# PythonOptimizers/pysparse

Measured on AMD Instinct MI355X. Metric: CSR SpMV GB/s (7-pt Poisson, % of 8 TB/s HBM peak) + PCG iters/s, higher is better.
Workload: dtype f64

## Files before the change

### pysparse_amd/csrc/psp_csr_kernels.h

```cpp

constexpr int kBlock = 256;


__global__ void build_chunk_table(int nrows, const int *__restrict__ ind, int target, int nchunks,
                                  int2 *__restrict__ tab) {
  int c = blockIdx.x * blockDim.x + threadIdx.x;
  if (c > nchunks) return;
  int r;
  if (c == nchunks) {
    r = nrows;
  } else {
    long want = (long)c * target;
    int lo = 0, hi = nrows;
    while (lo < hi) {
      int mid = lo + ((hi - lo) >> 1);
      if ((long)ind[mid] >= want)
        hi = mid;
      else
        lo = mid + 1;
    }
    r = lo;
  }
  tab[c] = make_int2(r, ind[r]);
}
// ... 1526 lines not shown
  const int blk = blk0 + vb * 4 + wid;
  const long r = (long)blk * kDiaRows + 2 * lane;
  double dsum = 0.0;
  if (blk < blk1 && r < nrows) {
    const uint2 mm = *reinterpret_cast<const uint2 *>(mask + r);
    const unsigned m0 = mm.x, m1 = mm.y;
    const double *vp = valT + (size_t)blk * NO * kDiaRows + 2 * lane;
    const long cmax = (long)ncols - 2;
    double a0 = 0.0, a1 = 0.0;
#pragma unroll
    for (int g = 0; g < NO; g += 8) {
      constexpr int G = 8;
      d2v v[G], xv[G];
      bool edge = false;
#pragma unroll
      for (int u = 0; u < G; ++u) {
        if (g + u < NO) {
          v[u] = ldg<true>(reinterpret_cast<const d2v *>(vp + (g + u) * kDiaRows));
          const long c = r + offs.o[g + u];
          const long cc = c < 0 ? 0 : (c > cmax ? cmax : c);
          const d2u t = *reinterpret_cast<const d2u *>(x + cc);
          xv[u].x = t.x;
          xv[u].y = t.y;
          edge |= cc != c;
        }
      }
      if (edge) {
#pragma unroll
        for (int u = 0; u < G; ++u) {
          if (g + u < NO) {
            const long c = r + offs.o[g + u];
            if (c < 0 || c > cmax) {
              xv[u].x = (c >= 0 && c < ncols) ? x[c] : 0.0;
              xv[u].y = (c + 1 >= 0 && c + 1 < ncols) ? x[c + 1] : 0.0;
            }
          }
        }
      }
#pragma unroll
      for (int u = 0; u < G; ++u) {
        if (g + u < NO) {
          const double t0 = a0 + v[u].x * xv[u].x;
          const double t1 = a1 + v[u].y * xv[u].y;
          a0 = ((m0 >> (g + u)) & 1u) ? t0 : a0;
          a1 = ((m1 >> (g + u)) & 1u) ? t1 : a1;
        }
      }
    }
    if (r + 1 < nrows) {
      d2u outu;
      outu.x = a0;
      outu.y = a1;
      __builtin_nontemporal_store(outu, reinterpret_cast<d2u *>(y + r));
      if (dotv) {
        const d2u u = *reinterpret_cast<const d2u *>(dotv + r);
        dsum += u.x * a0;
        dsum += u.y * a1;
      }
    } else {
      y[r] = a0;
      if (dotv) dsum += dotv[r] * a0;
    }
  }
  if (partials) {
    dsum = wave_sum(dsum);
    if (lane == 0) red[wid] = dsum;
    __syncthreads();
    if (threadIdx.x == 0) partials[blockIdx.x] = red[0] + red[1] + red[2] + red[3];
  }
}

__global__ __launch_bounds__(256) void csr_spmv_w4y(
    int blk0, int blk1, int nrows, int ncols, int stripe, int no, const int *__restrict__ offs,
    const double *__restrict__ valT, const unsigned long long *__restrict__ mask, const double *__restrict__ x,
    double *__restrict__ y, const double *__restrict__ dotv, double *__restrict__ partials,
    const int *__restrict__ skip) {
  if (skip && *skip) return;
  __shared__ double red[4];
  const int lane = threadIdx.x & 63;
  const int wid = __builtin_amdgcn_readfirstlane(threadIdx.x >> 6);
  int vb = (int)blockIdx.x;
  if (stripe > 0) {
    const int k = vb >> 3;
    vb = ((k / stripe) * 8 + (vb & 7)) * stripe + k % stripe;
  }
  const int blk = blk0 + vb * 4 + wid;
  const long r = (long)blk * kDiaRows + 2 * lane;
  double dsum = 0.0;
  if (blk < blk1 && r < nrows) {
    const ulonglong2 mm = *reinterpret_cast<const ulonglong2 *>(mask + r);
    const unsigned long long m0 = mm.x, m1 = mm.y;
    const double *vp = valT + (size_t)blk * no * kDiaRows + 2 * lane;
    const long cmax = (long)ncols - 2;
    double a0 = 0.0, a1 = 0.0;
    for (int g = 0; g < no; g += 8) {
      constexpr int G = 8;
      d2v v[G], xv[G];
      int og[G];
      bool edge = false;
#pragma unroll
      for (int u = 0; u < G; ++u) {
        const int gu = g + u < no ? g + u : no - 1;
        og[u] = offs[gu];
        v[u] = ldg<true>(reinterpret_cast<const d2v *>(vp + (size_t)gu * kDiaRows));
        const long c = r + og[u];
        const long cc = c < 0 ? 0 : (c > cmax ? cmax : c);
        const d2u t = *reinterpret_cast<const d2u *>(x + cc);
        xv[u].x = t.x;
        xv[u].y = t.y;
        edge |= cc != c;
      }
      if (edge) {
#pragma unroll
        for (int u = 0; u < G; ++u) {
          const long c = r + og[u];
          if (c < 0 || c > cmax) {
            xv[u].x = (c >= 0 && c < ncols) ? x[c] : 0.0;
            xv[u].y = (c + 1 >= 0 && c + 1 < ncols) ? x[c + 1] : 0.0;
          }
        }
      }
#pragma unroll
      for (int u = 0; u < G; ++u) {
        const double t0 = a0 + v[u].x * xv[u].x;
        const double t1 = a1 + v[u].y * xv[u].y;
        const bool live = g + u < no;
        a0 = (live && ((m0 >> (g + u)) & 1ull)) ? t0 : a0;
        a1 = (live && ((m1 >> (g + u)) & 1ull)) ? t1 : a1;
      }
    }
    if (r + 1 < nrows) {
      d2u outu;
      outu.x = a0;
      outu.y = a1;
      __builtin_nontemporal_store(outu, reinterpret_cast<d2u *>(y + r));
      if (dotv) {
        const d2u u = *reinterpret_cast<const d2u *>(dotv + r);
        dsum += u.x * a0;
        dsum += u.y * a1;
      }
    } else {
      y[r] = a0;
      if (dotv) dsum += dotv[r] * a0;
    }
  }
  if (partials) {
    dsum = wave_sum(dsum);
    if (lane == 0) red[wid] = dsum;
    __syncthreads();
    if (threadIdx.x == 0) partials[blockIdx.x] = red[0] + red[1] + red[2] + red[3];
  }
}

template <int NO, int PRE, bool XU = false>
__global__ __launch_bounds__(256) void csr_spmv_w4_pf(
    int nrows, int stripe, DiaOffs offs, const double *__restrict__ valT,
    const unsigned short *__restrict__ mask, const double *__restrict__ r, const double *__restrict__ dinv,
    double dc, const double *__restrict__ p_old, double *__restrict__ p_new, double *__restrict__ q,
    double beta, int first, double *__restrict__ partials, const psp::PcgDev *__restrict__ dstate,
    double *__restrict__ x = nullptr, double *__restrict__ scan_partials = nullptr) {
  double alpha_x = 0.0;
  bool xp = false;
  if (dstate) {
    if (dstate->status) return;
    beta = dstate->beta;
    first = dstate->it == 1;
    if constexpr (XU) {
      alpha_x = dstate->alpha_x;
      xp = dstate->xpend != 0;
    }
  }
  __shared__ double red[4];
  __shared__ double red2[4];
  double dmax = 0.0;
  const int lane = threadIdx.x & 63;
  const int wid = __builtin_amdgcn_readfirstlane(threadIdx.x >> 6);
  int vb = (int)blockIdx.x;
  if (stripe > 0) {
    const int k = vb >> 3;
    vb = ((k / stripe) * 8 + (vb & 7)) * stripe + k % stripe;
  }
  const int blk = vb * 4 + wid;
  const long row = (long)blk * kDiaRows + 2 * lane;
  double dsum = 0.0;
  if (row < nrows) {
    const unsigned mm = *reinterpret_cast<const unsigned *>(mask + row);
    const unsigned m0 = mm & 0xffffu, m1 = mm >> 16;
    const double *vp = valT + (size_t)blk * NO * kDiaRows + 2 * lane;
    d2v v[NO];
#pragma unroll
    for (int o = 0; o < NO; ++o) v[o] = ldg<true>(reinterpret_cast<const d2v *>(vp + o * kDiaRows));
    const long cmax = (long)nrows - 2;
    const long rc = row > cmax ? cmax : row;
    d2u rr[NO + 1], pp[NO + 1], dd[NO + 1];
    bool edge = rc != row;
#pragma unroll
    for (int o = 0; o <= NO; ++o) {
      const long c = o < NO ? row + offs.o[o] : row;
      const long cc = c < 0 ? 0 : (c > cmax ? cmax : c);
      rr[o] = *reinterpret_cast<const d2u *>(r + cc);
      if (!first) pp[o] = *reinterpret_cast<const d2u *>(p_old + cc);
      if constexpr (PRE == 1) dd[o] = *reinterpret_cast<const d2u *>(dinv + cc);
      edge |= cc != c;
    }
    if (edge) {
#pragma unroll
      for (int o = 0; o <= NO; ++o) {
        const long c = o < NO ? row + offs.o[o] : row;
        if (c < 0 || c > cmax) {
          const bool i0 = c >= 0 && c < nrows, i1 = c + 1 >= 0 && c + 1 < nrows;
          rr[o].x = i0 ? r[c] : 0.0;
          rr[o].y = i1 ? r[c + 1] : 0.0;
          if (!first) {
            pp[o].x = i0 ? p_old[c] : 0.0;
            pp[o].y = i1 ? p_old[c + 1] : 0.0;
          }
          if constexpr (PRE == 1) {
            dd[o].x = i0 ? dinv[c] : 0.0;
            dd[o].y = i1 ? dinv[c + 1] : 0.0;
          }
        }
      }
    }
    d2v pn[NO + 1];
#pragma unroll
    for (int o = 0; o <= NO; ++o) {
      double z0 = rr[o].x, z1 = rr[o].y;
      if constexpr (PRE == 1) {
        z0 = z0 * dd[o].x;
        z1 = z1 * dd[o].y;
      }
      if constexpr (PRE == 2) {
        z0 = z0 * dc;
        z1 = z1 * dc;
      }
      if (!first) {
        z0 = z0 + beta * pp[o].x;
        z1 = z1 + beta * pp[o].y;
      }
      pn[o].x = z0;
      pn[o].y = z1;
    }
    double a0 = 0.0, a1 = 0.0;
#pragma unroll
    for (int o = 0; o < NO; ++o) {
      const double t0 = a0 + v[o].x * pn[o].x;
      const double t1 = a1 + v[o].y * pn[o].y;
      a0 = ((m0 >> o) & 1u) ? t0 : a0;
      a1 = ((m1 >> o) & 1u) ? t1 : a1;
    }
    if (row + 1 < nrows) {
      d2u outq, outp;
      outq.x = a0;
      outq.y = a1;
      outp.x = pn[NO].x;
      outp.y = pn[NO].y;
      __builtin_nontemporal_store(outq, reinterpret_cast<d2u *>(q + row));
      *reinterpret_cast<d2u *>(p_new + row) = outp;
      dsum += pn[NO].x * a0;
      dsum += pn[NO].y * a1;
    } else {
      q[row] = a0;
      p_new[row] = pn[NO].x;
      dsum += pn[NO].x * a0;
    }
    if constexpr (XU) {
      if (xp) {
        const bool upd = alpha_x != 0.0;
        const bool two = row + 1 < nrows;
        d2u xx;
        if (two) {
          xx = *reinterpret_cast<const d2u *>(x + row);
        } else {
          xx.x = x[row];
          xx.y = 0.0;
        }
        const double po[2] = {pp[NO].x, pp[NO].y};
        double xv[2] = {xx.x, xx.y};
#pragma unroll
        for (int u = 0; u < 2; ++u) {
          if (u == 1 && !two) break;
          const double quot = fabs(alpha_x * po[u] / xv[u]);
          const double ddum = (xv[u] != 0.0) ? quot : ((po[u] != 0.0) ? 1.0 : 0.0);
          dmax = (ddum > dmax) ? ddum : dmax;
          if (upd) xv[u] = xv[u] + alpha_x * po[u];
        }
        if (two) {
          xx.x = xv[0];
          xx.y = xv[1];
          *reinterpret_cast<d2u *>(x + row) = xx;
        } else {
          x[row] = xv[0];
        }
      }
    }
  }
  if (partials) {
    dsum = wave_sum(dsum);
    if (lane == 0) red[wid] = dsum;
    if constexpr (XU) {
#pragma unroll
      for (int off = 32; off > 0; off >>= 1) {
        const double o = __shfl_down(dmax, off, 64);
        if (o > dmax) dmax = o;
      }
      if (lane == 0) red2[wid] = (1.0 + dmax != 1.0) ? 1.0 : 0.0;
    }
    __syncthreads();
    if (threadIdx.x == 0) {
      partials[blockIdx.x] = red[0] + red[1] + red[2] + red[3];
      if constexpr (XU) scan_partials[blockIdx.x] = red2[0] + red2[1] + red2[2] + red2[3];
    }
  }
}

template <int NO>
__global__ __launch_bounds__(256) void csr_spmv_w4_transp(
    int nrows, int ncols, DiaOffs offs, const double *__restrict__ valT, const unsigned short *__restrict__ mask,
    const double *__restrict__ x, double *__restrict__ y) {
  const long c = ((long)blockIdx.x * blockDim.x + threadIdx.x) * 2;
  if (c >= ncols) return;
  const long npad = ((long)nrows + kDiaRows - 1) / kDiaRows * kDiaRows;
  double a0 = 0.0, a1 = 0.0;
#pragma unroll
  for (int o = NO - 1; o >= 0; --o) {
    const long i0 = c - offs.o[o], i1 = i0 + 1;
    const bool in0 = i0 >= 0 && i0 < nrows, in1 = i1 >= 0 && i1 < nrows && c + 1 < ncols;
    const long j0 = i0 < 0 ? 0 : (i0 >= npad ? npad - 1 : i0), j1 = i1 < 0 ? 0 : (i1 >= npad ? npad - 1 : i1);
    const double v0 = valT[((size_t)(j0 / kDiaRows) * NO + o) * kDiaRows + (size_t)(j0 % kDiaRows)];
    const double v1 = valT[((size_t)(j1 / kDiaRows) * NO + o) * kDiaRows + (size_t)(j1 % kDiaRows)];
    const unsigned m0 = mask[j0], m1 = mask[j1];
    const double x0 = x[in0 ? i0 : 0], x1 = x[in1 ? i1 : 0];
    const double t0 = a0 + v0 * x0, t1 = a1 + v1 * x1;
    a0 = (in0 && ((m0 >> o) & 1u)) ? t0 : a0;
    a1 = (in1 && ((m1 >> o) & 1u)) ? t1 : a1;
  }
  y[c] = a0;
  if (c + 1 < ncols) y[c + 1] = a1;
}

__global__ void iota_int_kernel(int n, int *__restrict__ v) {
  for (int i = blockIdx.x * blockDim.x + threadIdx.x; i < n; i += gridDim.x * blockDim.x) v[i] = i;
}

__global__ void rows_of_nonzeros_kernel(int nrows, const int *__restrict__ ind, int *__restrict__ rows) {
  const int wave = (blockIdx.x * blockDim.x + threadIdx.x) >> 6, lane = threadIdx.x & 63;
  const int nwaves = (gridDim.x * blockDim.x) >> 6;
  for (int r = wave; r < nrows; r += nwaves)
    for (int k = ind[r] + lane; k < ind[r + 1]; k += 64) rows[k] = r;
}

__global__ void transp_gather_kernel(int nnz, const int *__restrict__ perm, const int *__restrict__ rows,
                                     const double *__restrict__ val, int *__restrict__ col_t,
                                     double *__restrict__ val_t) {
  for (int k = blockIdx.x * blockDim.x + threadIdx.x; k < nnz; k += gridDim.x * blockDim.x) {
    const int src = perm[k];
    col_t[k] = rows[src];
    val_t[k] = val[src];
  }
}

__global__ void transp_count_kernel(int nnz, int ncols, const int *__restrict__ col, int *__restrict__ cnt, int *bad) {
  for (long k = (long)blockIdx.x * blockDim.x + threadIdx.x; k < nnz; k += (long)gridDim.x * blockDim.x) {
    const int c = col[k];
    if (c < 0 || c >= ncols) *bad = 1;
    else atomicAdd(cnt + c, 1);
  }
}

__global__ void transp_slot_kernel(int nrows, const int *__restrict__ ind, const int *__restrict__ col,
                                   const int *__restrict__ tind, int *__restrict__ cursor,
                                   unsigned long long *__restrict__ key) {
  const int lane = threadIdx.x & 63;
  for (long r = (long)blockIdx.x * 4 + (threadIdx.x >> 6); r < nrows; r += (long)gridDim.x * 4)
    for (int k = ind[r] + lane; k < ind[r + 1]; k += 64) {
      const int c = col[k];
      const int at = tind[c] + atomicAdd(cursor + c, 1);
      key[at] = ((unsigned long long)(unsigned)r << 32) | (unsigned)k;
    }
}

__global__ void transp_maxlen_kernel(int ncols, const int *__restrict__ tind, int *maxlen) {
  int m = 0;
  for (int c = blockIdx.x * blockDim.x + threadIdx.x; c < ncols; c += gridDim.x * blockDim.x) m = max(m, tind[c + 1] - tind[c]);
#pragma unroll
  for (int off = 32; off > 0; off >>= 1) m = max(m, __shfl_down(m, off, 64));
  if ((threadIdx.x & 63) == 0 && m > 0) atomicMax(maxlen, m);
}

__global__ void transp_sort_kernel(int ncols, const int *__restrict__ tind, unsigned long long *__restrict__ key) {
  for (int c = blockIdx.x * blockDim.x + threadIdx.x; c < ncols; c += gridDim.x * blockDim.x) {
    const int b = tind[c], e = tind[c + 1];
    for (int i = b + 1; i < e; ++i) {
      const unsigned long long v = key[i];
// ... 87 lines not shown
```

### pysparse_amd/csrc/psp_csr_select.h

```cpp
namespace psp {

static int colmask() {
#ifdef PSP_TUNING
  static const int m = [] {
    const char *e = psp::tuning_env("PSP_SPMV_COLMASK");
    return e ? atoi(e) : -1;
  }();
  return m;
#else
  return -1;
#endif
}

static int spmv_stripe() {
  static const int m = [] {
    const char *e = psp::tuning_env("PSP_SPMV_STRIPE");
    return e ? atoi(e) : -1;
  }();
  return m;
}

static int w4_auto_stripe(const psp_csr *A) {
  if (A->sym_owner) return 32;
  int plane_wgs = 0;
// ... 227 lines not shown
__global__ __launch_bounds__(256) void grid_wrap_check_kernel(int n, int nx, int ny, const unsigned short *__restrict__ mask,
                                                              int *__restrict__ bad) {
  int found = 0;
  for (long r = (long)blockIdx.x * blockDim.x + threadIdx.x; r < n; r += (long)gridDim.x * blockDim.x) {
    const unsigned m = mask[r];
    const int i = (int)(r % nx), j = (int)((r / nx) % ny);
    if (((m >> 2) & 1u) && i == 0) found = 1;
    if (((m >> 4) & 1u) && i == nx - 1) found = 1;
    if (((m >> 1) & 1u) && j == 0) found = 1;
    if (((m >> 5) & 1u) && j == ny - 1) found = 1;
  }
  if (found) atomicAdd(bad, 1);
}

__global__ __launch_bounds__(256) void w4_value_range_kernel(int n, int no, const double *__restrict__ valT,
                                                             const unsigned short *__restrict__ mask, double *__restrict__ out) {
  __shared__ double smin[4][16], smax[4][16];
  double lo[16], hi[16];
  for (int o = 0; o < 16; ++o) {
    lo[o] = INFINITY;
    hi[o] = -INFINITY;
  }
  for (long r = (long)blockIdx.x * blockDim.x + threadIdx.x; r < n; r += (long)gridDim.x * blockDim.x) {
    const unsigned m = mask[r];
    const double *vp = valT + (size_t)(r / kDiaRows) * no * kDiaRows + (size_t)(r % kDiaRows);
    for (int o = 0; o < no; ++o)
      if ((m >> o) & 1u) {
        const double v = vp[(size_t)o * kDiaRows];
        lo[o] = v < lo[o] ? v : lo[o];
        hi[o] = v > hi[o] ? v : hi[o];
        if (!(v == v)) hi[o] = INFINITY, lo[o] = -INFINITY;
      }
  }
  const int lane = threadIdx.x & 63, wid = threadIdx.x >> 6;
  for (int o = 0; o < no; ++o) {
    double a = lo[o], b = hi[o];
    for (int off = 32; off > 0; off >>= 1) {
      const double a2 = __shfl_down(a, off, 64), b2 = __shfl_down(b, off, 64);
      a = a2 < a ? a2 : a;
      b = b2 > b ? b2 : b;
    }
    if (lane == 0) {
      smin[wid][o] = a;
      smax[wid][o] = b;
    }
  }
  __syncthreads();
  if ((int)threadIdx.x < no) {
    const int o = threadIdx.x;
    double a = smin[0][o], b = smax[0][o];
    for (int w = 1; w < 4; ++w) {
      a = smin[w][o] < a ? smin[w][o] : a;
      b = smax[w][o] > b ? smax[w][o] : b;
    }
    out[((size_t)blockIdx.x * no + o) * 2] = a;
    out[((size_t)blockIdx.x * no + o) * 2 + 1] = b;
  }
}

int csr_w4_view(const psp_csr *A, W4View *out, int *available) {
  *available = 0;
  Variant v = decode_variant(A->variant);
  if (A->w4_only) v.w4 = true;
  if (!v.w4 || A->nparts || A->multi || A->host || A->nrows != A->ncols || A->nrows < 2) return PSP_OK;
  psp::CsrExtra *ex;
  PSP_TRY(ensure_w4(A, &ex));
  if (ex->dia_state != 1 || ex->dia_no > 9 || !ex->dia_mask) return PSP_OK;
  out->no = ex->dia_no;
  for (int i = 0; i < 12; ++i) out->offs[i] = i < ex->dia_no ? ex->dia_offs.o[i] : 0;
  out->valT = ex->dia_val;
  out->mask = ex->dia_mask;
  out->stripe = w4_stripe(A, v);
  out->grid = w4_grid((A->nrows + kDiaRows - 1) / kDiaRows, out->stripe);
  out->grid3[0] = out->grid3[1] = out->grid3[2] = 0;
  if (ex->dia_no == 7) {
    const int *o = out->offs;
    const int s1 = o[5], s2 = o[6];
    if (ex->grid_state < 0) {
      ex->grid_state = 0;
      if (o[3] == 0 && o[4] == 1 && o[2] == -1 && o[1] == -s1 && o[0] == -s2 && s1 >= 2 && s2 % s1 == 0 && s2 / s1 >= 2 &&
          A->nrows % s2 == 0 && A->nrows / s2 >= 2) {
        int *bad = nullptr;
        PSP_HIP(hipMalloc((void **)&bad, sizeof(int)));
        PSP_HIP(hipMemsetAsync(bad, 0, sizeof(int), stream()));
        hipLaunchKernelGGL(grid_wrap_check_kernel, dim3(std::min((A->nrows + 255) / 256, 4096)), dim3(256), 0, stream(),
                           A->nrows, s1, s2 / s1, ex->dia_mask, bad);
        int hbad = 1;
        const hipError_t e1 = hipMemcpyAsync(&hbad, bad, sizeof(int), hipMemcpyDeviceToHost, stream());
        const hipError_t e2 = hipStreamSynchronize(stream());
        (void)hipFree(bad);
        if (e1 != hipSuccess || e2 != hipSuccess) return fail(PSP_ENODEV, "csr_w4_view: grid check failed");
        if (hbad == 0) {
          ex->grid_state = 1;
          ex->grid_nx = s1;
          ex->grid_ny = s2 / s1;
        }
      }
    }
    if (ex->grid_state == 1) {
      out->grid3[0] = ex->grid_nx;
      out->grid3[1] = ex->grid_ny;
      out->grid3[2] = A->nrows / (ex->grid_nx * ex->grid_ny);
    }
  }
  out->constv = 0;
  if (ex->dia_no <= 12) {
    if (ex->constv_state < 0) {
      ex->constv_state = 0;
      const int no = ex->dia_no, blocks = std::min((A->nrows + 255) / 256, 512);
      double *d = nullptr;
      PSP_HIP(hipMalloc((void **)&d, sizeof(double) * 2 * no * blocks));
      hipLaunchKernelGGL(w4_value_range_kernel, dim3(blocks), dim3(256), 0, stream(), A->nrows, no, ex->dia_val, ex->dia_mask, d);
      std::vector<double> h((size_t)2 * no * blocks);
      const hipError_t e1 = hipMemcpyAsync(h.data(), d, sizeof(double) * h.size(), hipMemcpyDeviceToHost, stream());
      const hipError_t e2 = hipStreamSynchronize(stream());
      (void)hipFree(d);
      if (e1 != hipSuccess || e2 != hipSuccess) return fail(PSP_ENODEV, "csr_w4_view: value range pass failed");
      bool all = true;
      for (int o = 0; o < no && all; ++o) {
        double lo = INFINITY, hi = -INFINITY;
        for (int b = 0; b < blocks; ++b) {
          lo = std::min(lo, h[((size_t)b * no + o) * 2]);
          hi = std::max(hi, h[((size_t)b * no + o) * 2 + 1]);
        }
        if (!(lo == hi) || std::signbit(lo) != std::signbit(hi)) all = false;
        ex->constv[o] = lo;
      }
      if (all) ex->constv_state = 1;
    }
    if (ex->constv_state == 1) {
      out->constv = 1;
      for (int o = 0; o < 12; ++o) out->cval[o] = o < ex->dia_no ? ex->constv[o] : 0.0;
    }
  }
  *available = 1;
  return PSP_OK;
}

int csr_spmv_pfx_launch(const psp_csr *A, const double *r, const double *dinv, const double *p_old, double *p_new,
                        double *q, double *x, double *partials, int *nparts, const PcgDev *dstate, int *available) {
  *available = 0;
  Variant v = decode_variant(A->variant);
  if (!v.w4 || A->nparts || A->sym_owner || A->nrows != A->ncols || A->nrows < 2 || !dstate || !partials) return PSP_OK;
  psp::CsrExtra *ex;
  PSP_TRY(ensure_w4(A, &ex));
  if (ex->dia_state != 1 || ex->dia_no > 8) return PSP_OK;
  const int stripe = w4_stripe(A, v);
  const int nblk = (A->nrows + kDiaRows - 1) / kDiaRows;
  const int grid = w4_grid(nblk, stripe);
  if (grid > kMaxParts) return PSP_OK;
  double dc = 0.0;
  const int pre = !dinv ? 0 : (dinv_constant(dinv, A->nrows, &dc) ? 2 : 1);
  double *scan = partials + 2 * (size_t)kMaxParts;
#define PSP_PFX(NO, PRE)                                                                                    \
  hipLaunchKernelGGL((csr_spmv_w4_pf<NO, PRE, true>), dim3(grid), dim3(256), 0, stream(), A->nrows, stripe, \
                     ex->dia_offs, ex->dia_val, ex->dia_mask, r, dinv, dc, p_old, p_new, q, 0.0, 0, partials, dstate, x, scan)
#define PSP_PFX_NO(NO)                \
  case NO:                            \
    if (pre == 0) PSP_PFX(NO, 0);     \
    else if (pre == 1) PSP_PFX(NO, 1); \
    else PSP_PFX(NO, 2);              \
    break
  switch (ex->dia_no) {
    PSP_PFX_NO(1); PSP_PFX_NO(2); PSP_PFX_NO(3); PSP_PFX_NO(4); PSP_PFX_NO(5); PSP_PFX_NO(6); PSP_PFX_NO(7); PSP_PFX_NO(8);
    default:
      return PSP_OK;
  }
#undef PSP_PFX_NO
#undef PSP_PFX
  PSP_LAUNCH_CHECK();
  *nparts = grid;
  *available = 1;
  return PSP_OK;
}

bool csr_spmv_has_skip(const psp_csr *A) {
  if (A->nparts) {
    for (int p = 0; p < A->nparts; ++p)
      if (A->parts[p]->nrows && !csr_spmv_has_skip(A->parts[p])) return false;
    return true;
  }
  Variant v = decode_variant(A->variant);
  if (A->w4_only) v.w4 = true;
  if (v.w4 && A->sym_owner) {
    psp_sss *S = const_cast<psp_sss *>(A->sym_owner);
    if (ensure_sss_w4(S) != PSP_OK) return false;
    if (S->w4_state == 1) return true;
  }
  if (v.w4) {
    psp::CsrExtra *ex;
    if (ensure_w4(A, &ex) != PSP_OK) return false;
    if (ex->dia_state == 1) return true;
  }
  if (!v.w2 || A->max_row_nnz > v.tile / 2) return false;
  ChunkTable *t;
  if (get_chunk_table(const_cast<psp_csr *>(A), v.tile, &t) != PSP_OK) return false;
  if (ensure_rowoff(A, t) != PSP_OK) return false;
  return t->np != 0;
}

int csr_reordered_view(const psp_csr *A, psp_csr **R, const int **perm, const int **inv) {
  *R = nullptr;
  psp::setup_mark(nullptr);
  Variant v = decode_variant(A->variant);
  if (A->nparts || A->w4_only || A->no_reorder || !(v.w1 && v.w2 && v.w3) || A->nrows != A->ncols ||
      A->max_row_nnz > v.tile / 2 || v.tile != 1024)
    return PSP_OK;
  if (v.w4) {
    if (A->sym_owner) {
      psp_sss *S = const_cast<psp_sss *>(A->sym_owner);
      PSP_TRY(ensure_sss_w4(S));
      if (S->w4_state == 1) return PSP_OK;
    }
    psp::CsrExtra *ex;
    PSP_TRY(ensure_w4(A, &ex));
    if (ex->dia_state == 1) return PSP_OK;
  }
  psp::setup_mark("first use: index-free (w4) layouts tried");
  ChunkTable *t;
  PSP_TRY(get_chunk_table(const_cast<psp_csr *>(A), v.tile, &t));
  PSP_TRY(ensure_rowoff(A, t));
  if (t->np == 0) return PSP_OK;
  psp::setup_mark("first use: chunk table + row offsets");
  PSP_TRY(ensure_w3(A, t));
  psp::setup_mark("first use: w3 tables on the stored numbering");
  psp::CsrExtra *exs = nullptr;
  int mode = 0;
  PSP_TRY(pick_scattered(A, t, &exs, &mode));
  if (mode != 1) return PSP_OK;
  exs->reordered->variant = A->variant;
  *R = exs->reordered;
  *perm = exs->perm;
  *inv = exs->inv;
  return PSP_OK;
}

int csr_spmv_launch(const psp_csr *A, const double *x, double *y, const double *dotv,
                    double *partials, int *nparts, const int *skip) {
  Workspace *w;
  PSP_TRY(workspace(&w));
  psp::setup_mark(nullptr);
  if (A->nparts) {
    double *tmp = w->partials + (size_t)(kSlots - 1) * kMaxParts;
    if (partials && (partials == tmp || (long)A->nparts * kFold > kMaxParts))
      return fail(PSP_EINVAL, "csr_spmv_launch: partitioned matrix needs a partial-sum slot other than the last");
    for (int p = 0; p < A->nparts; ++p) {
      const psp_csr *P = A->parts[p];
      if (P->nrows == 0) continue;
      const int r0 = A->part_row0[p];
      int np = 0;
      PSP_TRY(csr_spmv_launch(P, x, y + r0, (partials && dotv) ? dotv + r0 : nullptr, partials ? tmp : nullptr, &np,
                              skip));
      if (partials) {
        hipLaunchKernelGGL(fold_partials_kernel, dim3(kFold / 16), dim3(256), 0, stream(), tmp, np,
                           partials + (size_t)p * kFold, kFold);
        PSP_LAUNCH_CHECK();
      }
    }
    if (nparts) *nparts = A->nparts * kFold;
    return PSP_OK;
  }
  Variant v = decode_variant(A->variant);
  if (A->w4_only) v.w4 = true;
  if (v.w4 && A->sym_owner) {
    psp_sss *S = const_cast<psp_sss *>(A->sym_owner);
    PSP_TRY(ensure_sss_w4(S));
    if (S->w4_state == 1) {
      const int stripe = w4_stripe(A, v);
      const int nblk = (S->n + kDiaRows - 1) / kDiaRows;
      const int grid = w4_grid(nblk, stripe);
      double *pbuf = partials;
      if (partials && grid > kMaxParts) {
        psp::CsrExtra *ex;
        {
          std::lock_guard<std::mutex> lk(g_extra_mu);
          ex = &g_extra[A];
        }
        PSP_TRY(ensure_big_partials(ex, grid));
        pbuf = ex->big_partials;
      }
      PSP_TRY(launch_sss_w4(S, stripe, x, y, dotv, pbuf, skip, grid));
      int np = grid;
      if (pbuf != partials) {
        np = kFold;
        hipLaunchKernelGGL(fold_partials_kernel, dim3(np / 16), dim3(256), 0, stream(), pbuf, grid,
                           partials, np);
        PSP_LAUNCH_CHECK();
      }
      if (nparts) *nparts = np;
      return PSP_OK;
    }
  }
  if (v.w4) {
    psp::CsrExtra *ex;
    PSP_TRY(ensure_w4(A, &ex));
    if (ex->dia_state == 1) {
      const int stripe = w4_stripe(A, v);
      const int nblk = (A->nrows + kDiaRows - 1) / kDiaRows;
      const int grid = w4_grid(nblk, stripe);
      double *pbuf = partials;
      if (partials && grid > kMaxParts) {
        PSP_TRY(ensure_big_partials(ex, grid));
        pbuf = ex->big_partials;
      }
      PSP_TRY(launch_w4(A, ex, stripe, 0, nblk, x, y, dotv, pbuf, skip, grid));
      int np = grid;
      if (pbuf != partials) {
        np = kFold;
        hipLaunchKernelGGL(fold_partials_kernel, dim3(np / 16), dim3(256), 0, stream(), pbuf, grid,
                           partials, np);
        PSP_LAUNCH_CHECK();
      }
      if (nparts) *nparts = np;
      return PSP_OK;
    }
  }
  if (A->w4_only) return fail(PSP_EINVAL, "this operator exists only in the w4 layout (psp_csr_poisson_big)");
  if ((v.wave || v.w1) && A->max_row_nnz > v.tile / 2) {
    v.wave = v.w1 = v.w2 = false;
    v.tile = 2048;
    v.vec = 4;
// ... 563 lines not shown
```

### pysparse_amd/csrc/psp_csr_tables.h

```cpp

struct ChunkTable {
  int tile = 0;
  int target = 0;
  int nchunks = 0;
  int2 *tab = nullptr;
  int max_rows = -1;
  int np = 0;
  unsigned short *rowoff = nullptr;
  int nb = -1;
  int max_blocks = 0;
  int outliers = 0;
  int *blist = nullptr;
  unsigned short *col16 = nullptr;
  int nb6 = -1;
  int direct6 = 0;
  int *blist6 = nullptr;
  int nu = -1;
  int max_cols = 0;
  int *ulist = nullptr;
  unsigned short *colu = nullptr;
  int sched_state = -1;
  int sched_grid = 0;
  int *perm = nullptr;
  int half_band = 0;
// ... 226 lines not shown
    (void)hipGetLastError();
    t->blist6 = nullptr;
    return PSP_OK;
  }
  hipLaunchKernelGGL(build_w3_kernel<64>, dim3(t->nchunks), dim3(64), 0, stream(), t->nchunks, t->target, 1, t->tab,
                     A->col, t->blist6, (unsigned short *)nullptr, d_max);
  PSP_LAUNCH_CHECK();
  PSP_HIP(hipStreamSynchronize(stream()));
  t->nb6 = 64;
  return PSP_OK;
}

static int ensure_w5(const psp_csr *A, ChunkTable *t) {
  std::lock_guard<std::mutex> lk(g_extra_mu);
  if (t->nu >= 0) return PSP_OK;
  t->nu = 0;
  static const bool off = [] {
    const char *e = psp::tuning_env("PSP_SPMV_W5");
    return e && atoi(e) == 0;
  }();
  if (off || t->tile != 1024 || t->np == 0 || A->nnz == 0) return PSP_OK;
  ScratchDev max_mem;
  PSP_HIP(hipMalloc(&max_mem.p, sizeof(int)));
  int *d_max = (int *)max_mem.p;
  PSP_HIP(hipMemsetAsync(d_max, 0, sizeof(int), stream()));
  hipLaunchKernelGGL((build_w3_kernel<1024, 0>), dim3(t->nchunks), dim3(64), 0, stream(), t->nchunks, t->target, 0,
                     t->tab, A->col, (int *)nullptr, (unsigned short *)nullptr, d_max);
  PSP_LAUNCH_CHECK();
  int mc = 0;
  PSP_HIP(hipMemcpyAsync(&mc, d_max, sizeof(int), hipMemcpyDeviceToHost, stream()));
  PSP_HIP(hipStreamSynchronize(stream()));
  t->max_cols = mc;
  int nu = 0;
  if (mc <= 256) nu = 256;
  else if (mc <= 384) nu = 384;
  else if (mc <= 512) nu = 512;
  if (nu == 0) return PSP_OK;
  hipError_t e1 = hipMalloc((void **)&t->ulist, sizeof(int) * (size_t)t->nchunks * nu);
  hipError_t e2 = hipMalloc((void **)&t->colu, sizeof(unsigned short) * (size_t)t->nchunks * 1024);
  if (e1 != hipSuccess || e2 != hipSuccess) {
    (void)hipGetLastError();
    if (e1 == hipSuccess) (void)hipFree(t->ulist);
    if (e2 == hipSuccess) (void)hipFree(t->colu);
    t->ulist = nullptr;
    t->colu = nullptr;
    return PSP_OK;
  }
#define PSP_BUILD_W5(NU)                                                                              \
  hipLaunchKernelGGL((build_w3_kernel<NU, 0>), dim3(t->nchunks), dim3(64), 0, stream(), t->nchunks,    \
                     t->target, 1, t->tab, A->col, t->ulist, t->colu, d_max)
  if (nu == 256) PSP_BUILD_W5(256);
  else if (nu == 384) PSP_BUILD_W5(384);
  else PSP_BUILD_W5(512);
#undef PSP_BUILD_W5
  PSP_LAUNCH_CHECK();
  PSP_HIP(hipStreamSynchronize(stream()));
  t->nu = nu;
  return PSP_OK;
}

__global__ void band_kernel(int nrows, const int *__restrict__ ind, const int *__restrict__ col,
                            int *__restrict__ out) {
  int lo = 0x7fffffff, hi = -0x7fffffff;
  for (int r = blockIdx.x * blockDim.x + threadIdx.x; r < nrows; r += gridDim.x * blockDim.x) {
    const int a = ind[r], b = ind[r + 1];
    if (b > a) {
      lo = min(lo, col[a] - r);
      hi = max(hi, col[b - 1] - r);
    }
  }
#pragma unroll
  for (int off = 32; off > 0; off >>= 1) {
    lo = min(lo, __shfl_down(lo, off, 64));
    hi = max(hi, __shfl_down(hi, off, 64));
  }
  if ((threadIdx.x & 63) == 0) {
    atomicMin(out, lo);
    atomicMax(out + 1, hi);
  }
}

static int sched_strip_rows() {
  static const int v = [] {
    const char *e = psp::tuning_env("PSP_SPMV_STRIP_ROWS");
    return e ? atoi(e) : 0;
  }();
  return v;
}

static int ensure_schedule(const psp_csr *A, ChunkTable *t) {
  std::lock_guard<std::mutex> lk(g_extra_mu);
  if (t->sched_state >= 0) return PSP_OK;
  t->sched_state = 0;
  const bool forced = A->sched_strip_rows >= 0;
  const int strip_rows = forced ? A->sched_strip_rows : sched_strip_rows();
  const int nwg = (t->nchunks + 3) / 4;
  if (strip_rows <= 0 || A->nrows < 1 || (!forced && nwg < 4096)) return PSP_OK;
  int *d_band;
  PSP_HIP(hipMalloc((void **)&d_band, 2 * sizeof(int)));
  const int init[2] = {0x7fffffff, -0x7fffffff};
  PSP_HIP(hipMemcpyAsync(d_band, init, sizeof(init), hipMemcpyHostToDevice, stream()));
  hipLaunchKernelGGL(band_kernel, dim3(std::min((A->nrows + 255) / 256, 4096)), dim3(256), 0, stream(),
                     A->nrows, A->ind, A->col, d_band);
  PSP_LAUNCH_CHECK();
  int band[2];
  PSP_HIP(hipMemcpyAsync(band, d_band, sizeof(band), hipMemcpyDeviceToHost, stream()));
  PSP_HIP(hipStreamSynchronize(stream()));
  PSP_HIP(hipFree(d_band));
  if (band[1] < band[0]) return PSP_OK;
  const long D = ((long)band[1] - band[0]) / 2;
  t->half_band = (int)D;
  if (D < 1 || (!forced && (D < 4L * strip_rows || D > A->nrows / 3))) return PSP_OK;
  long nstrips = (D + strip_rows / 2) / strip_rows;
  nstrips = (nstrips + 7) / 8 * 8;
  const double w = (double)D / (double)nstrips;
  std::vector<int2> tab((size_t)t->nchunks + 1);
  PSP_HIP(hipMemcpy(tab.data(), t->tab, sizeof(int2) * tab.size(), hipMemcpyDeviceToHost));
  struct Key {
    int strip, period, wg;
  };
  std::vector<Key> keys((size_t)nwg);
  for (int g = 0; g < nwg; ++g) {
    const long r0 = tab[(size_t)g * 4].x;
    long strip = (long)((double)(r0 % D) / w);
    if (strip >= nstrips) strip = nstrips - 1;
    keys[g] = {(int)strip, (int)(r0 / D), g};
  }
  std::sort(keys.begin(), keys.end(), [](const Key &a, const Key &b) {
    if (a.strip != b.strip) return a.strip < b.strip;
    if (a.period != b.period) return a.period < b.period;
    return a.wg < b.wg;
  });
  const int per = (nwg + 7) / 8;
  const int grid = per * 8;
  std::vector<int> perm((size_t)grid, -1);
  for (int j = 0; j < 8; ++j)
    for (int p = 0; p < per; ++p) {
      const long src = (long)j * per + p;
      if (src < nwg) perm[(size_t)p * 8 + j] = keys[(size_t)src].wg;
    }
  PSP_HIP(hipMalloc((void **)&t->perm, sizeof(int) * (size_t)grid));
  PSP_HIP(hipMemcpy(t->perm, perm.data(), sizeof(int) * (size_t)grid, hipMemcpyHostToDevice));
  t->sched_grid = grid;
  t->sched_state = 1;
  return PSP_OK;
}

static int ensure_w4(const psp_csr *A, psp::CsrExtra **out) {
  std::lock_guard<std::mutex> lk(g_extra_mu);
  psp::CsrExtra &ex = g_extra[A];
  *out = &ex;
  if (ex.dia_state >= 0) return PSP_OK;
  ex.dia_state = 0;
  static const bool off = [] {
    const char *e = psp::tuning_env("PSP_SPMV_W4");
    return e && atoi(e) == 0;
  }();
  if (off || A->nrows < 1 || A->ncols < 2 || A->nnz < 1 || A->max_row_nnz > kDiaMaxOffs) return PSP_OK;
  ScratchDev tab_mem;
  PSP_HIP(hipMalloc(&tab_mem.p, (kDiaTable + 1) * sizeof(int)));
  int *d_tab = (int *)tab_mem.p;
  int init[kDiaTable + 1];
  for (int i = 0; i < kDiaTable; ++i) init[i] = kDiaEmpty;
  init[kDiaTable] = 0;
  PSP_HIP(hipMemcpyAsync(d_tab, init, sizeof(init), hipMemcpyHostToDevice, stream()));
  hipLaunchKernelGGL(dia_offsets_kernel, dim3(std::min((A->nrows + 255) / 256, 8192)), dim3(256), 0, stream(),
                     A->nrows, A->ind, A->col, d_tab, d_tab + kDiaTable);
  PSP_LAUNCH_CHECK();
  int tab[kDiaTable + 1];
  PSP_HIP(hipMemcpyAsync(tab, d_tab, sizeof(tab), hipMemcpyDeviceToHost, stream()));
  PSP_HIP(hipStreamSynchronize(stream()));
  if (tab[kDiaTable]) return PSP_OK;
  std::vector<int> offs;
  for (int i = 0; i < kDiaTable; ++i)
    if (tab[i] != kDiaEmpty) offs.push_back(tab[i]);
  if (offs.empty() || (int)offs.size() > kDiaMaxOffs) return PSP_OK;
  std::sort(offs.begin(), offs.end());
  const int no = (int)offs.size();
  const size_t nblk = ((size_t)A->nrows + kDiaRows - 1) / kDiaRows;
  const double slots = (double)nblk * kDiaRows * no;
  if (slots * 8.0 > 11.0 * (double)A->nnz) return PSP_OK;
  for (int i = 0; i < kDiaMaxOffs; ++i) ex.dia_offs.o[i] = i < no ? offs[i] : 0;
  const size_t nval = nblk * kDiaRows * no;
  const bool m32 = no > 16 && no <= 32, m64 = no > 32;
  const size_t nmask = nblk * kDiaRows + 2;
  hipError_t e1 = hipMalloc((void **)&ex.dia_val, sizeof(double) * nval);
  if (e1 != hipSuccess) {
    (void)hipGetLastError();
    (void)psp_trim();
    e1 = hipMalloc((void **)&ex.dia_val, sizeof(double) * nval);
  }
  hipError_t e2 = m64   ? hipMalloc((void **)&ex.dia_mask64, sizeof(unsigned long long) * nmask)
                  : m32 ? hipMalloc((void **)&ex.dia_mask32, sizeof(unsigned) * nmask)
                        : hipMalloc((void **)&ex.dia_mask, sizeof(unsigned short) * nmask);
  hipError_t e3 = m64 ? hipMalloc((void **)&ex.dia_offs_dev, sizeof(int) * kDiaMaxOffs) : hipSuccess;
  if (e3 == hipSuccess && m64)
    e3 = hipMemcpyAsync(ex.dia_offs_dev, ex.dia_offs.o, sizeof(int) * kDiaMaxOffs, hipMemcpyHostToDevice, stream());
  if (e1 != hipSuccess || e2 != hipSuccess || e3 != hipSuccess) {
    (void)hipGetLastError();
    if (e1 == hipSuccess) (void)hipFree(ex.dia_val);
    if (e2 == hipSuccess) (void)hipFree(m64 ? (void *)ex.dia_mask64 : m32 ? (void *)ex.dia_mask32 : (void *)ex.dia_mask);
    if (ex.dia_offs_dev) (void)hipFree(ex.dia_offs_dev);
    ex.dia_val = nullptr;
    ex.dia_mask = nullptr;
    ex.dia_mask32 = nullptr;
    ex.dia_mask64 = nullptr;
    ex.dia_offs_dev = nullptr;
    return PSP_OK;
  }
  PSP_HIP(hipMemsetAsync(ex.dia_val, 0, sizeof(double) * nval, stream()));
  const int bgrid = std::min((A->nrows + 255) / 256, 65536);
  if (m64) {
    PSP_HIP(hipMemsetAsync(ex.dia_mask64, 0, sizeof(unsigned long long) * nmask, stream()));
    hipLaunchKernelGGL(dia_build_kernel<unsigned long long>, dim3(bgrid), dim3(256), 0, stream(), A->nrows, no,
                       ex.dia_offs, A->ind, A->col, A->val, ex.dia_val, ex.dia_mask64);
  } else if (m32) {
    PSP_HIP(hipMemsetAsync(ex.dia_mask32, 0, sizeof(unsigned) * nmask, stream()));
    hipLaunchKernelGGL(dia_build_kernel<unsigned>, dim3(bgrid), dim3(256), 0, stream(), A->nrows, no, ex.dia_offs,
                       A->ind, A->col, A->val, ex.dia_val, ex.dia_mask32);
  } else {
    PSP_HIP(hipMemsetAsync(ex.dia_mask, 0, sizeof(unsigned short) * nmask, stream()));
    hipLaunchKernelGGL(dia_build_kernel<unsigned short>, dim3(bgrid), dim3(256), 0, stream(), A->nrows, no,
                       ex.dia_offs, A->ind, A->col, A->val, ex.dia_val, ex.dia_mask);
  }
  PSP_LAUNCH_CHECK();
  PSP_HIP(hipStreamSynchronize(stream()));
  ex.dia_no = no;
  ex.dia_state = 1;
  return PSP_OK;
}

static bool w4_dot_reload() {
  const char *e = psp::tuning_env("PSP_W4_DOT_RELOAD");
  return e && atoi(e) != 0;
}

static int launch_w4(const psp_csr *A, const psp::CsrExtra *ex, int stripe, int b0, int b1, const double *x,
                     double *y, const double *dotv, double *pbuf, const int *skip, int grid, int use_div = 0,
                     double xdiv = 1.0, const double *xdiv_dev = nullptr) {
  if (use_div && ex->dia_no > 16) return fail(PSP_EINVAL, "csr_spmv_w4x has no scaled form");
  const int flags = (A->variant >= 0 ? A->variant : 0) >> 23 & 3;
  int dot_slot = -1;
  if (dotv && ex->dia_no <= 16 && !w4_dot_reload()) {
    const intptr_t diff = (intptr_t)dotv - (intptr_t)x;
    if (diff % (intptr_t)sizeof(double) == 0)
      for (int k = 0; k < ex->dia_no; ++k)
        if ((intptr_t)ex->dia_offs.o[k] == diff / (intptr_t)sizeof(double)) dot_slot = k;
  }
#define PSP_W4_F(NO, NTL, NTS)                                                                       \
  hipLaunchKernelGGL((csr_spmv_w4<NO, NTL, NTS>), dim3(grid), dim3(256), 0, stream(), b0, b1, A->nrows, \
                     A->ncols, stripe, ex->dia_offs, ex->dia_val, ex->dia_mask, x, y, dotv, pbuf, skip,  \
                     use_div, xdiv, xdiv_dev, dot_slot)
#define PSP_W4(NO)                                                                                   \
  case NO:                                                                                           \
    if (flags == 0) PSP_W4_F(NO, true, true);                                                        \
    else if (flags == 1) PSP_W4_F(NO, false, true);                                                  \
    else if (flags == 2) PSP_W4_F(NO, true, false);                                                  \
    else PSP_W4_F(NO, false, false);                                                                 \
    break
  switch (ex->dia_no) {
    PSP_W4(1); PSP_W4(2); PSP_W4(3); PSP_W4(4); PSP_W4(5); PSP_W4(6); PSP_W4(7); PSP_W4(8);
    PSP_W4(9); PSP_W4(10); PSP_W4(11); PSP_W4(12); PSP_W4(13); PSP_W4(14); PSP_W4(15); PSP_W4(16);
#define PSP_W4X(NO)                                                                                  \
  case NO:                                                                                           \
    hipLaunchKernelGGL((csr_spmv_w4x<NO>), dim3(grid), dim3(256), 0, stream(), b0, b1, A->nrows,      \
                       A->ncols, stripe, ex->dia_offs, ex->dia_val, ex->dia_mask32, x, y, dotv, pbuf, \
                       skip);                                                                        \
    break
    PSP_W4X(17); PSP_W4X(18); PSP_W4X(19); PSP_W4X(20); PSP_W4X(21); PSP_W4X(22); PSP_W4X(23); PSP_W4X(24);
    PSP_W4X(25); PSP_W4X(26); PSP_W4X(27); PSP_W4X(28); PSP_W4X(29); PSP_W4X(30); PSP_W4X(31); PSP_W4X(32);
#undef PSP_W4X
    default:
      if (ex->dia_no > 32 && ex->dia_no <= kDiaMaxOffs && ex->dia_mask64) {
        hipLaunchKernelGGL(csr_spmv_w4y, dim3(grid), dim3(256), 0, stream(), b0, b1, A->nrows, A->ncols, stripe,
                           ex->dia_no, ex->dia_offs_dev, ex->dia_val, ex->dia_mask64, x, y, dotv, pbuf, skip);
        break;
      }
      return fail(PSP_EINVAL, "csr_spmv_w4: %d offsets", ex->dia_no);
  }
#undef PSP_W4
#undef PSP_W4_F
  PSP_LAUNCH_CHECK();
  return PSP_OK;
}

static int w4_grid(int nblocks, int stripe) {
  int grid = (nblocks + 3) / 4;
  if (stripe > 0) grid = (grid + 8 * stripe - 1) / (8 * stripe) * (8 * stripe);
  return grid;
}

static int ensure_big_partials(psp::CsrExtra *ex, int cap) {
  std::lock_guard<std::mutex> lk(g_extra_mu);
  if (ex->big_cap < cap) {
    if (ex->big_partials) (void)hipFree(ex->big_partials);
    ex->big_partials = nullptr;
    ex->big_cap = 0;
    PSP_HIP(hipMalloc((void **)&ex->big_partials, sizeof(double) * (size_t)cap));
    ex->big_cap = cap;
  }
  return PSP_OK;
}

static std::mutex g_sss_mu;
static int ensure_sss_w4(psp_sss *S) {
  std::lock_guard<std::mutex> lk(g_sss_mu);
  if (S->w4_state >= 0) return PSP_OK;
  S->w4_state = 0;
  static const bool off = [] {
    const char *e = psp::tuning_env("PSP_SSS_W4");
    return e && atoi(e) == 0;
  }();
  if (off || S->n < 2 || S->nnz_lower < 1) return PSP_OK;
  ScratchDev tab_mem;
  PSP_HIP(hipMalloc(&tab_mem.p, (kDiaTable + 1) * sizeof(int)));
  int *d_tab = (int *)tab_mem.p;
  int init[kDiaTable + 1];
  for (int i = 0; i < kDiaTable; ++i) init[i] = kDiaEmpty;
  init[kDiaTable] = 0;
  PSP_HIP(hipMemcpyAsync(d_tab, init, sizeof(init), hipMemcpyHostToDevice, stream()));
  hipLaunchKernelGGL(dia_offsets_kernel, dim3(std::min((S->n + 255) / 256, 8192)), dim3(256), 0, stream(), S->n,
                     S->ind, S->col, d_tab, d_tab + kDiaTable);
  PSP_LAUNCH_CHECK();
  int tab[kDiaTable + 1];
  PSP_HIP(hipMemcpyAsync(tab, d_tab, sizeof(tab), hipMemcpyDeviceToHost, stream()));
  PSP_HIP(hipStreamSynchronize(stream()));
  if (tab[kDiaTable]) return PSP_OK;
  std::vector<int> offs;
  for (int i = 0; i < kDiaTable; ++i)
    if (tab[i] != kDiaEmpty) offs.push_back(tab[i]);
  if (offs.empty() || offs.size() > 8) return PSP_OK;
  std::sort(offs.begin(), offs.end());
  const int nol = (int)offs.size();
  const size_t nblk = ((size_t)S->n + kDiaRows - 1) / kDiaRows;
// ... 380 lines not shown
```

Baseline: 6155.

## Reuse centre-row p values via lane shuffles for the -1/0/+1 diagonals in fused PCG SpMV

When the DIA offsets contain -1, 0 and +1 consecutively, the fused p-update/SpMV kernel skips the separate gathers of r, p_old and dinv for the two neighbour diagonals. It rebuilds those values from the centre pair with wave shuffles plus one halo load at lanes 0 and 63, which cuts redundant cache and memory loads per row. The p_old loads are also made unconditional and the `first` check moved into a small helper, so the first iteration does some extra loads. A new PSP_SPMV_W4=2 mode bypasses the DIA fill-ratio check, and the launcher gains template instantiations for each possible centre index.

```diff
diff --git a/pysparse_amd/csrc/psp_csr_kernels.h b/pysparse_amd/csrc/psp_csr_kernels.h
--- a/pysparse_amd/csrc/psp_csr_kernels.h
+++ b/pysparse_amd/csrc/psp_csr_kernels.h
@@ -1702,13 +1702,14 @@
   }
 }
 
-template <int NO, int PRE, bool XU = false>
+template <int NO, int PRE, bool XU = false, int C = -1>
 __global__ __launch_bounds__(256) void csr_spmv_w4_pf(
     int nrows, int stripe, DiaOffs offs, const double *__restrict__ valT,
     const unsigned short *__restrict__ mask, const double *__restrict__ r, const double *__restrict__ dinv,
     double dc, const double *__restrict__ p_old, double *__restrict__ p_new, double *__restrict__ q,
     double beta, int first, double *__restrict__ partials, const psp::PcgDev *__restrict__ dstate,
     double *__restrict__ x = nullptr, double *__restrict__ scan_partials = nullptr) {
+  static_assert(C < 0 || (C >= 1 && C + 1 < NO), "the centre needs both neighbours");
   double alpha_x = 0.0;
   bool xp = false;
   if (dstate) {
@@ -1746,25 +1747,36 @@
     bool edge = rc != row;
 #pragma unroll
     for (int o = 0; o <= NO; ++o) {
+      if (C >= 0 && o >= C - 1 && o <= C + 1) continue;
       const long c = o < NO ? row + offs.o[o] : row;
       const long cc = c < 0 ? 0 : (c > cmax ? cmax : c);
       rr[o] = *reinterpret_cast<const d2u *>(r + cc);
-      if (!first) pp[o] = *reinterpret_cast<const d2u *>(p_old + cc);
+      pp[o] = *reinterpret_cast<const d2u *>(p_old + cc);
       if constexpr (PRE == 1) dd[o] = *reinterpret_cast<const d2u *>(dinv + cc);
       edge |= cc != c;
     }
+    double hr = 0.0, hp = 0.0, hd = 0.0;
+    if constexpr (C >= 0) {
+      if (lane == 0 || lane == 63) {
+        const long hc = lane == 0 ? row - 1 : row + 2;
+        if (hc >= 0 && hc < nrows) {
+          hr = r[hc];
+          hp = p_old[hc];
+          if constexpr (PRE == 1) hd = dinv[hc];
+        }
+      }
+    }
     if (edge) {
 #pragma unroll
       for (int o = 0; o <= NO; ++o) {
+        if (C >= 0 && o >= C - 1 && o <= C + 1) continue;
         const long c = o < NO ? row + offs.o[o] : row;
         if (c < 0 || c > cmax) {
           const bool i0 = c >= 0 && c < nrows, i1 = c + 1 >= 0 && c + 1 < nrows;
           rr[o].x = i0 ? r[c] : 0.0;
           rr[o].y = i1 ? r[c + 1] : 0.0;
-          if (!first) {
-            pp[o].x = i0 ? p_old[c] : 0.0;
-            pp[o].y = i1 ? p_old[c + 1] : 0.0;
-          }
+          pp[o].x = i0 ? p_old[c] : 0.0;
+          pp[o].y = i1 ? p_old[c + 1] : 0.0;
           if constexpr (PRE == 1) {
             dd[o].x = i0 ? dinv[c] : 0.0;
             dd[o].y = i1 ? dinv[c + 1] : 0.0;
@@ -1772,24 +1784,27 @@
         }
       }
     }
+    auto form = [&](double z, double d, double po) {
+      if constexpr (PRE == 1) z = z * d;
+      if constexpr (PRE == 2) z = z * dc;
+      return first ? z : z + beta * po;
+    };
     d2v pn[NO + 1];
 #pragma unroll
     for (int o = 0; o <= NO; ++o) {
-      double z0 = rr[o].x, z1 = rr[o].y;
-      if constexpr (PRE == 1) {
-        z0 = z0 * dd[o].x;
-        z1 = z1 * dd[o].y;
-      }
-      if constexpr (PRE == 2) {
-        z0 = z0 * dc;
-        z1 = z1 * dc;
-      }
-      if (!first) {
-        z0 = z0 + beta * pp[o].x;
-        z1 = z1 + beta * pp[o].y;
-      }
-      pn[o].x = z0;
-      pn[o].y = z1;
+      if (C >= 0 && o >= C - 1 && o <= C + 1) continue;
+      pn[o].x = form(rr[o].x, PRE == 1 ? dd[o].x : 0.0, pp[o].x);
+      pn[o].y = form(rr[o].y, PRE == 1 ? dd[o].y : 0.0, pp[o].y);
+    }
+    if constexpr (C >= 0) {
+      const double ph = form(hr, hd, hp);
+      const double up = __shfl_up(pn[NO].y, 1, 64);
+      const double dn = __shfl_down(pn[NO].x, 1, 64);
+      pn[C - 1].x = lane == 0 ? ph : up;
+      pn[C - 1].y = pn[NO].x;
+      pn[C] = pn[NO];
+      pn[C + 1].x = pn[NO].y;
+      pn[C + 1].y = (row + 2 >= nrows) ? 0.0 : (lane == 63 ? ph : dn);
     }
     double a0 = 0.0, a1 = 0.0;
 #pragma unroll
diff --git a/pysparse_amd/csrc/psp_csr_select.h b/pysparse_amd/csrc/psp_csr_select.h
--- a/pysparse_amd/csrc/psp_csr_select.h
+++ b/pysparse_amd/csrc/psp_csr_select.h
@@ -403,14 +403,28 @@
   double dc = 0.0;
   const int pre = !dinv ? 0 : (dinv_constant(dinv, A->nrows, &dc) ? 2 : 1);
   double *scan = partials + 2 * (size_t)kMaxParts;
-#define PSP_PFX(NO, PRE)                                                                                    \
-  hipLaunchKernelGGL((csr_spmv_w4_pf<NO, PRE, true>), dim3(grid), dim3(256), 0, stream(), A->nrows, stripe, \
+  int c = -1;
+  for (int i = 1; i + 1 < ex->dia_no; ++i)
+    if (ex->dia_offs.o[i] == 0 && ex->dia_offs.o[i - 1] == -1 && ex->dia_offs.o[i + 1] == 1) c = i;
+#define PSP_PFX(NO, PRE, C)                                                                                    \
+  hipLaunchKernelGGL((csr_spmv_w4_pf<NO, PRE, true, C>), dim3(grid), dim3(256), 0, stream(), A->nrows, stripe, \
                      ex->dia_offs, ex->dia_val, ex->dia_mask, r, dinv, dc, p_old, p_new, q, 0.0, 0, partials, dstate, x, scan)
-#define PSP_PFX_NO(NO)                \
-  case NO:                            \
-    if (pre == 0) PSP_PFX(NO, 0);     \
-    else if (pre == 1) PSP_PFX(NO, 1); \
-    else PSP_PFX(NO, 2);              \
+#define PSP_PFX_C(NO, C)               \
+  if (pre == 0) PSP_PFX(NO, 0, C);     \
+  else if (pre == 1) PSP_PFX(NO, 1, C); \
+  else PSP_PFX(NO, 2, C)
+#define PSP_PFX_CASE(NO, C) \
+  case C:                   \
+    PSP_PFX_C(NO, (C < NO - 1 ? C : -1)); \
+    break
+#define PSP_PFX_NO(NO)                                                                                        \
+  case NO:                                                                                                    \
+    switch (c < NO - 1 ? c : -1) {                                                                            \
+      PSP_PFX_CASE(NO, 1); PSP_PFX_CASE(NO, 2); PSP_PFX_CASE(NO, 3); PSP_PFX_CASE(NO, 4); PSP_PFX_CASE(NO, 5); \
+      PSP_PFX_CASE(NO, 6);                                                                                    \
+      default:                                                                                                \
+        PSP_PFX_C(NO, -1);                                                                                    \
+    }                                                                                                         \
     break
   switch (ex->dia_no) {
     PSP_PFX_NO(1); PSP_PFX_NO(2); PSP_PFX_NO(3); PSP_PFX_NO(4); PSP_PFX_NO(5); PSP_PFX_NO(6); PSP_PFX_NO(7); PSP_PFX_NO(8);
@@ -418,6 +432,8 @@
       return PSP_OK;
   }
 #undef PSP_PFX_NO
+#undef PSP_PFX_CASE
+#undef PSP_PFX_C
 #undef PSP_PFX
   PSP_LAUNCH_CHECK();
   *nparts = grid;
diff --git a/pysparse_amd/csrc/psp_csr_tables.h b/pysparse_amd/csrc/psp_csr_tables.h
--- a/pysparse_amd/csrc/psp_csr_tables.h
+++ b/pysparse_amd/csrc/psp_csr_tables.h
@@ -402,10 +402,11 @@
   *out = &ex;
   if (ex.dia_state >= 0) return PSP_OK;
   ex.dia_state = 0;
-  static const bool off = [] {
+  static const int mode = [] {
     const char *e = psp::tuning_env("PSP_SPMV_W4");
-    return e && atoi(e) == 0;
-  }();
+    return e ? atoi(e) : 1;
+  }();
+  const bool off = mode == 0;
   if (off || A->nrows < 1 || A->ncols < 2 || A->nnz < 1 || A->max_row_nnz > kDiaMaxOffs) return PSP_OK;
   ScratchDev tab_mem;
   PSP_HIP(hipMalloc(&tab_mem.p, (kDiaTable + 1) * sizeof(int)));
@@ -429,7 +430,7 @@
   const int no = (int)offs.size();
   const size_t nblk = ((size_t)A->nrows + kDiaRows - 1) / kDiaRows;
   const double slots = (double)nblk * kDiaRows * no;
-  if (slots * 8.0 > 11.0 * (double)A->nnz) return PSP_OK;
+  if (mode != 2 && slots * 8.0 > 11.0 * (double)A->nnz) return PSP_OK;
   for (int i = 0; i < kDiaMaxOffs; ++i) ex.dia_offs.o[i] = i < no ? offs[i] : 0;
   const size_t nval = nblk * kDiaRows * no;
   const bool m32 = no > 16 && no <= 32, m64 = no > 32;
```

After: 6159 (median of 5 runs). Within noise of the previous version (+0.1%).
